# loicland/superpoint_graph

Hardware: NVIDIA H100
Metric: spg_train_step_edges_plus_points_per_sec (higher is better)
Workload: dtype f32

## Files before the change

### superpoint_graph_b200/csrc/tc_common.cuh

```cuda
#pragma once
#include <cuda_runtime.h>
#include <stdint.h>

namespace spg {

__device__ __forceinline__ uint32_t smem_u32(const void* p) {
    return (uint32_t)__cvta_generic_to_shared(p);
}

__device__ __forceinline__ uint32_t to_tf32(float v) {
    return (__float_as_uint(v) + 0x1000u) & 0xffffe000u;
}

__device__ __forceinline__ void mbar_init(uint32_t bar, uint32_t count) {
    asm volatile("mbarrier.init.shared::cta.b64 [%0], %1;" ::"r"(bar), "r"(count));
}

__device__ __forceinline__ void mbar_wait(uint32_t bar, uint32_t parity) {
    asm volatile(
        "{\n\t"
        ".reg .pred P1;\n\t"
        "WAIT_LOOP:\n\t"
        "mbarrier.try_wait.parity.shared::cta.b64 P1, [%0], %1;\n\t"
        "@P1 bra WAIT_DONE;\n\t"
        "bra WAIT_LOOP;\n\t"
        "WAIT_DONE:\n\t"
        "}" ::"r"(bar), "r"(parity)
        : "memory");
}

__device__ __forceinline__ void mbar_arrive(uint32_t bar) {
    asm volatile("mbarrier.arrive.shared::cta.b64 _, [%0];" ::"r"(bar) : "memory");
}

__device__ __forceinline__ void mbar_expect_tx(uint32_t bar, uint32_t bytes) {
    asm volatile("mbarrier.arrive.expect_tx.shared::cta.b64 _, [%0], %1;" ::"r"(bar), "r"(bytes) : "memory");
}

__device__ __forceinline__ uint64_t wg_desc_k_sw128(uint32_t saddr) {
    return (uint64_t)((saddr >> 4) & 0x3FFFu) | ((uint64_t)1 << 16) | ((uint64_t)64 << 32) | ((uint64_t)1 << 62);
}

__device__ __forceinline__ uint32_t sw128_off(int row, int c16) {
    return (uint32_t)((row >> 3) * 1024 + (row & 7) * 128 + ((c16 ^ (row & 7)) << 4));
}

__device__ __forceinline__ void wg_fence() { asm volatile("wgmma.fence.sync.aligned;" ::: "memory"); }
__device__ __forceinline__ void wg_commit() { asm volatile("wgmma.commit_group.sync.aligned;" ::: "memory"); }
template <int N>
__device__ __forceinline__ void wg_wait() {
    asm volatile("wgmma.wait_group.sync.aligned %0;" ::"n"(N) : "memory");
}

template <int R>
__device__ __forceinline__ void wg_reg_fence(float (&d)[R]) {
#pragma unroll
    for (int i = 0; i < R; ++i) asm volatile("" : "+f"(d[i])::"memory");
}

template <int N>
__device__ __forceinline__ void wgmma_tf32(float (&d)[N / 2], uint64_t da, uint64_t db, uint32_t acc);
template <int N>
__device__ __forceinline__ void wgmma_bf16(float (&d)[N / 2], uint64_t da, uint64_t db, uint32_t acc);

template <>
__device__ __forceinline__ void wgmma_tf32<16>(float (&d)[8], uint64_t da, uint64_t db, uint32_t acc) {
    asm volatile(
        "{\n\t.reg .pred p;\n\tsetp.ne.b32 p, %10, 0;\n\t"
        "wgmma.mma_async.sync.aligned.m64n16k8.f32.tf32.tf32 {%0, %1, %2, %3, %4, %5, %6, %7}, %8, %9, p, 1, 1;\n\t}"
        : "+f"(d[0]), "+f"(d[1]), "+f"(d[2]), "+f"(d[3]), "+f"(d[4]), "+f"(d[5]), "+f"(d[6]), "+f"(d[7])
        : "l"(da), "l"(db), "r"(acc));
}

template <>
__device__ __forceinline__ void wgmma_tf32<32>(float (&d)[16], uint64_t da, uint64_t db, uint32_t acc) {
    asm volatile(
        "{\n\t.reg .pred p;\n\tsetp.ne.b32 p, %18, 0;\n\t"
        "wgmma.mma_async.sync.aligned.m64n32k8.f32.tf32.tf32 {%0, %1, %2, %3, %4, %5, %6, %7, %8, %9, %10, %11, %12, %13, %14, %15}, %16, %17, p, 1, 1;\n\t}"
        : "+f"(d[0]), "+f"(d[1]), "+f"(d[2]), "+f"(d[3]), "+f"(d[4]), "+f"(d[5]), "+f"(d[6]), "+f"(d[7]), "+f"(d[8]), "+f"(d[9]), "+f"(d[10]), "+f"(d[11]), "+f"(d[12]), "+f"(d[13]), "+f"(d[14]), "+f"(d[15])
        : "l"(da), "l"(db), "r"(acc));
}

template <>
__device__ __forceinline__ void wgmma_tf32<64>(float (&d)[32], uint64_t da, uint64_t db, uint32_t acc) {
    asm volatile(
        "{\n\t.reg .pred p;\n\tsetp.ne.b32 p, %34, 0;\n\t"
        "wgmma.mma_async.sync.aligned.m64n64k8.f32.tf32.tf32 {%0, %1, %2, %3, %4, %5, %6, %7, %8, %9, %10, %11, %12, %13, %14, %15, %16, %17, %18, %19, %20, %21, %22, %23, %24, %25, %26, %27, %28, %29, %30, %31}, %32, %33, p, 1, 1;\n\t}"
        : "+f"(d[0]), "+f"(d[1]), "+f"(d[2]), "+f"(d[3]), "+f"(d[4]), "+f"(d[5]), "+f"(d[6]), "+f"(d[7]), "+f"(d[8]), "+f"(d[9]), "+f"(d[10]), "+f"(d[11]), "+f"(d[12]), "+f"(d[13]), "+f"(d[14]), "+f"(d[15]), "+f"(d[16]), "+f"(d[17]), "+f"(d[18]), "+f"(d[19]), "+f"(d[20]), "+f"(d[21]), "+f"(d[22]), "+f"(d[23]), "+f"(d[24]), "+f"(d[25]), "+f"(d[26]), "+f"(d[27]), "+f"(d[28]), "+f"(d[29]), "+f"(d[30]), "+f"(d[31])
        : "l"(da), "l"(db), "r"(acc));
}

template <>
__device__ __forceinline__ void wgmma_tf32<128>(float (&d)[64], uint64_t da, uint64_t db, uint32_t acc) {
    asm volatile(
        "{\n\t.reg .pred p;\n\tsetp.ne.b32 p, %66, 0;\n\t"
        "wgmma.mma_async.sync.aligned.m64n128k8.f32.tf32.tf32 {%0, %1, %2, %3, %4, %5, %6, %7, %8, %9, %10, %11, %12, %13, %14, %15, %16, %17, %18, %19, %20, %21, %22, %23, %24, %25, %26, %27, %28, %29, %30, %31, %32, %33, %34, %35, %36, %37, %38, %39, %40, %41, %42, %43, %44, %45, %46, %47, %48, %49, %50, %51, %52, %53, %54, %55, %56, %57, %58, %59, %60, %61, %62, %63}, %64, %65, p, 1, 1;\n\t}"
        : "+f"(d[0]), "+f"(d[1]), "+f"(d[2]), "+f"(d[3]), "+f"(d[4]), "+f"(d[5]), "+f"(d[6]), "+f"(d[7]), "+f"(d[8]), "+f"(d[9]), "+f"(d[10]), "+f"(d[11]), "+f"(d[12]), "+f"(d[13]), "+f"(d[14]), "+f"(d[15]), "+f"(d[16]), "+f"(d[17]), "+f"(d[18]), "+f"(d[19]), "+f"(d[20]), "+f"(d[21]), "+f"(d[22]), "+f"(d[23]), "+f"(d[24]), "+f"(d[25]), "+f"(d[26]), "+f"(d[27]), "+f"(d[28]), "+f"(d[29]), "+f"(d[30]), "+f"(d[31]), "+f"(d[32]), "+f"(d[33]), "+f"(d[34]), "+f"(d[35]), "+f"(d[36]), "+f"(d[37]), "+f"(d[38]), "+f"(d[39]), "+f"(d[40]), "+f"(d[41]), "+f"(d[42]), "+f"(d[43]), "+f"(d[44]), "+f"(d[45]), "+f"(d[46]), "+f"(d[47]), "+f"(d[48]), "+f"(d[49]), "+f"(d[50]), "+f"(d[51]), "+f"(d[52]), "+f"(d[53]), "+f"(d[54]), "+f"(d[55]), "+f"(d[56]), "+f"(d[57]), "+f"(d[58]), "+f"(d[59]), "+f"(d[60]), "+f"(d[61]), "+f"(d[62]), "+f"(d[63])
        : "l"(da), "l"(db), "r"(acc));
}

template <>
__device__ __forceinline__ void wgmma_bf16<32>(float (&d)[16], uint64_t da, uint64_t db, uint32_t acc) {
    asm volatile(
        "{\n\t.reg .pred p;\n\tsetp.ne.b32 p, %18, 0;\n\t"
        "wgmma.mma_async.sync.aligned.m64n32k16.f32.bf16.bf16 {%0, %1, %2, %3, %4, %5, %6, %7, %8, %9, %10, %11, %12, %13, %14, %15}, %16, %17, p, 1, 1, 0, 0;\n\t}"
        : "+f"(d[0]), "+f"(d[1]), "+f"(d[2]), "+f"(d[3]), "+f"(d[4]), "+f"(d[5]), "+f"(d[6]), "+f"(d[7]), "+f"(d[8]), "+f"(d[9]), "+f"(d[10]), "+f"(d[11]), "+f"(d[12]), "+f"(d[13]), "+f"(d[14]), "+f"(d[15])
        : "l"(da), "l"(db), "r"(acc));
}

template <>
__device__ __forceinline__ void wgmma_bf16<64>(float (&d)[32], uint64_t da, uint64_t db, uint32_t acc) {
    asm volatile(
        "{\n\t.reg .pred p;\n\tsetp.ne.b32 p, %34, 0;\n\t"
        "wgmma.mma_async.sync.aligned.m64n64k16.f32.bf16.bf16 {%0, %1, %2, %3, %4, %5, %6, %7, %8, %9, %10, %11, %12, %13, %14, %15, %16, %17, %18, %19, %20, %21, %22, %23, %24, %25, %26, %27, %28, %29, %30, %31}, %32, %33, p, 1, 1, 0, 0;\n\t}"
        : "+f"(d[0]), "+f"(d[1]), "+f"(d[2]), "+f"(d[3]), "+f"(d[4]), "+f"(d[5]), "+f"(d[6]), "+f"(d[7]), "+f"(d[8]), "+f"(d[9]), "+f"(d[10]), "+f"(d[11]), "+f"(d[12]), "+f"(d[13]), "+f"(d[14]), "+f"(d[15]), "+f"(d[16]), "+f"(d[17]), "+f"(d[18]), "+f"(d[19]), "+f"(d[20]), "+f"(d[21]), "+f"(d[22]), "+f"(d[23]), "+f"(d[24]), "+f"(d[25]), "+f"(d[26]), "+f"(d[27]), "+f"(d[28]), "+f"(d[29]), "+f"(d[30]), "+f"(d[31])
        : "l"(da), "l"(db), "r"(acc));
}

template <>
__device__ __forceinline__ void wgmma_bf16<128>(float (&d)[64], uint64_t da, uint64_t db, uint32_t acc) {
    asm volatile(
        "{\n\t.reg .pred p;\n\tsetp.ne.b32 p, %66, 0;\n\t"
        "wgmma.mma_async.sync.aligned.m64n128k16.f32.bf16.bf16 {%0, %1, %2, %3, %4, %5, %6, %7, %8, %9, %10, %11, %12, %13, %14, %15, %16, %17, %18, %19, %20, %21, %22, %23, %24, %25, %26, %27, %28, %29, %30, %31, %32, %33, %34, %35, %36, %37, %38, %39, %40, %41, %42, %43, %44, %45, %46, %47, %48, %49, %50, %51, %52, %53, %54, %55, %56, %57, %58, %59, %60, %61, %62, %63}, %64, %65, p, 1, 1, 0, 0;\n\t}"
        : "+f"(d[0]), "+f"(d[1]), "+f"(d[2]), "+f"(d[3]), "+f"(d[4]), "+f"(d[5]), "+f"(d[6]), "+f"(d[7]), "+f"(d[8]), "+f"(d[9]), "+f"(d[10]), "+f"(d[11]), "+f"(d[12]), "+f"(d[13]), "+f"(d[14]), "+f"(d[15]), "+f"(d[16]), "+f"(d[17]), "+f"(d[18]), "+f"(d[19]), "+f"(d[20]), "+f"(d[21]), "+f"(d[22]), "+f"(d[23]), "+f"(d[24]), "+f"(d[25]), "+f"(d[26]), "+f"(d[27]), "+f"(d[28]), "+f"(d[29]), "+f"(d[30]), "+f"(d[31]), "+f"(d[32]), "+f"(d[33]), "+f"(d[34]), "+f"(d[35]), "+f"(d[36]), "+f"(d[37]), "+f"(d[38]), "+f"(d[39]), "+f"(d[40]), "+f"(d[41]), "+f"(d[42]), "+f"(d[43]), "+f"(d[44]), "+f"(d[45]), "+f"(d[46]), "+f"(d[47]), "+f"(d[48]), "+f"(d[49]), "+f"(d[50]), "+f"(d[51]), "+f"(d[52]), "+f"(d[53]), "+f"(d[54]), "+f"(d[55]), "+f"(d[56]), "+f"(d[57]), "+f"(d[58]), "+f"(d[59]), "+f"(d[60]), "+f"(d[61]), "+f"(d[62]), "+f"(d[63])
        : "l"(da), "l"(db), "r"(acc));
}


}
```

### superpoint_graph_b200/csrc/tc_dw.cu

```cuda
#include "common.cuh"
#include "tc_common.cuh"

namespace spg {

constexpr int DW_THREADS = 256;
constexpr int DW_PTS = 32;

struct DwArgs {
    const float* dY;
    int64_t lddy;
    const float* P;
    int64_t ldp;
    const float *p_scale, *p_shift;
    int p_relu;
    float* partial;
    int64_t M;
    int64_t pts_per_cta;
};

template <int CO, int CI>
__global__ void __launch_bounds__(DW_THREADS, 1) tc_dw_kernel(const DwArgs p) {
    constexpr int WM = CO >= 128 ? CO / 2 : 64;
    constexpr int WN = CO >= 128 ? CI : CI / 2;
    constexpr int MSUB = WM / 64;
    constexpr int A_BYTES = CO * DW_PTS * 4;
    constexpr int B_BYTES = CI * DW_PTS * 4;
    constexpr int STAGE_BYTES = 2 * A_BYTES + 2 * B_BYTES;
    static_assert(CO % 64 == 0 && CI % 32 == 0 && CI <= 128 && CO <= 256, "shape");
    constexpr int A_F4 = CO * DW_PTS / 4 / DW_THREADS;
    constexpr int B_F4 = CI * DW_PTS / 4 / DW_THREADS;

    extern __shared__ __align__(1024) uint8_t smem_raw[];
    uint8_t* smem = reinterpret_cast<uint8_t*>((reinterpret_cast<uintptr_t>(smem_raw) + 1023) & ~(uintptr_t)1023);

    const int t = threadIdx.x;
    const int warp = t >> 5, lane = t & 31;
    const int g = warp >> 2, wl = warp & 3;
    SPG_PDL_ENTRY();

    const int64_t m_beg = (int64_t)blockIdx.x * p.pts_per_cta;
    const int64_t m_end = min(p.M, m_beg + p.pts_per_cta);
    const int nchunks = m_beg < m_end ? (int)((m_end - m_beg + DW_PTS - 1) / DW_PTS) : 0;
    const bool pro = p.p_scale || p.p_shift || p.p_relu;

    auto coord = [](int i, int c4s, int& pt, int& c4) {
        const int wi = i >> 5, l = i & 31;
        pt = (wi & 3) * 8 + (l & 7);
        c4 = (wi >> 2) * 4 + (l >> 3);
        (void)c4s;
    };
    float4 ra[A_F4], rb[B_F4];
    auto load_chunk = [&](int ch) {
        const int64_t mrow = m_beg + (int64_t)ch * DW_PTS;
#pragma unroll
        for (int j = 0; j < A_F4; ++j) {
            int pt, c4;
            coord(t + DW_THREADS * j, CO / 4, pt, c4);
            ra[j] = (mrow + pt < m_end)
                        ? __ldg(reinterpret_cast<const float4*>(p.dY + (mrow + pt) * p.lddy + c4 * 4))
                        : make_float4(0.f, 0.f, 0.f, 0.f);
        }
#pragma unroll
        for (int j = 0; j < B_F4; ++j) {
            int pt, c4;
            coord(t + DW_THREADS * j, CI / 4, pt, c4);
            rb[j] = (mrow + pt < m_end)
                        ? __ldg(reinterpret_cast<const float4*>(p.P + (mrow + pt) * p.ldp + c4 * 4))
                        : make_float4(0.f, 0.f, 0.f, 0.f);
        }
    };
    auto split_store = [&](uint8_t* hi_base, uint8_t* lo_base, int pt, int c4, float4 v) {
        const float vv[4] = {v.x, v.y, v.z, v.w};
#pragma unroll
        for (int e = 0; e < 4; ++e) {
            const uint32_t off = sw128_off(4 * c4 + e, pt >> 2) + (uint32_t)(pt & 3) * 4u;
            const uint32_t hi = to_tf32(vv[e]);
            *reinterpret_cast<uint32_t*>(hi_base + off) = hi;
            *reinterpret_cast<uint32_t*>(lo_base + off) = to_tf32(vv[e] - __uint_as_float(hi));
        }
    };

    float acc[MSUB][WN / 2];
#pragma unroll
    for (int m = 0; m < MSUB; ++m)
#pragma unroll
        for (int i = 0; i < WN / 2; ++i) acc[m][i] = 0.f;
    const int row_g = CO >= 128 ? g * WM : 0;
    const int col_g = CO >= 128 ? 0 : g * WN;

    if (nchunks > 0) load_chunk(0);
    for (int ch = 0; ch < nchunks; ++ch) {
        const int s = ch & 1;
        uint8_t* stage = smem + (size_t)s * STAGE_BYTES;
        uint8_t* a_hi = stage;
        uint8_t* a_lo = stage + A_BYTES;
        uint8_t* b_hi = stage + 2 * A_BYTES;
        uint8_t* b_lo = b_hi + B_BYTES;
        wg_wait<1>();
        wg_reg_fence(acc[0]);
        if (MSUB > 1) wg_reg_fence(acc[MSUB - 1]);
        __syncthreads();
        const int64_t mrow = m_beg + (int64_t)ch * DW_PTS;
#pragma unroll
        for (int j = 0; j < A_F4; ++j) {
            int pt, c4;
            coord(t + DW_THREADS * j, CO / 4, pt, c4);
            split_store(a_hi, a_lo, pt, c4, ra[j]);
        }
#pragma unroll
        for (int j = 0; j < B_F4; ++j) {
            int pt, c4;
            coord(t + DW_THREADS * j, CI / 4, pt, c4);
            float4 v = rb[j];
            if (pro && (mrow + pt < m_end)) {
                float4 sc = make_float4(1.f, 1.f, 1.f, 1.f), sh = make_float4(0.f, 0.f, 0.f, 0.f);
                if (p.p_scale) sc = __ldg(reinterpret_cast<const float4*>(p.p_scale + c4 * 4));
                if (p.p_shift) sh = __ldg(reinterpret_cast<const float4*>(p.p_shift + c4 * 4));
                v.x = fmaf(v.x, sc.x, sh.x);
                v.y = fmaf(v.y, sc.y, sh.y);
                v.z = fmaf(v.z, sc.z, sh.z);
                v.w = fmaf(v.w, sc.w, sh.w);
                if (p.p_relu) {
                    v.x = fmaxf(v.x, 0.f);
                    v.y = fmaxf(v.y, 0.f);
                    v.z = fmaxf(v.z, 0.f);
                    v.w = fmaxf(v.w, 0.f);
                }
            }
            split_store(b_hi, b_lo, pt, c4, v);
        }
        asm volatile("fence.proxy.async.shared::cta;" ::: "memory");
        __syncthreads();
        {
            const uint32_t ah = smem_u32(a_hi) + (uint32_t)row_g * 128u, al = smem_u32(a_lo) + (uint32_t)row_g * 128u;
            const uint32_t bh = smem_u32(b_hi) + (uint32_t)col_g * 128u, bl = smem_u32(b_lo) + (uint32_t)col_g * 128u;
#pragma unroll
            for (int m = 0; m < MSUB; ++m) wg_reg_fence(acc[m]);
            wg_fence();
#pragma unroll
            for (int kb = 0; kb < DW_PTS / 8; ++kb) {
                const uint64_t dbh = wg_desc_k_sw128(bh + kb * 32), dbl = wg_desc_k_sw128(bl + kb * 32);
#pragma unroll
                for (int m = 0; m < MSUB; ++m) {
                    const uint64_t dah = wg_desc_k_sw128(ah + m * 64 * 128 + kb * 32);
                    const uint64_t dal = wg_desc_k_sw128(al + m * 64 * 128 + kb * 32);
                    wgmma_tf32<WN>(acc[m], dah, dbh, 1u);
                    wgmma_tf32<WN>(acc[m], dal, dbh, 1u);
                    wgmma_tf32<WN>(acc[m], dah, dbl, 1u);
                }
            }
            wg_commit();
        }
        if (ch + 1 < nchunks) load_chunk(ch + 1);
    }
    wg_wait<0>();
#pragma unroll
    for (int m = 0; m < MSUB; ++m) wg_reg_fence(acc[m]);

    float* out = p.partial + (int64_t)blockIdx.x * CO * CI;
    const int r = lane >> 2, cq = 2 * (lane & 3);
#pragma unroll
    for (int m = 0; m < MSUB; ++m) {
        const int row = row_g + m * 64 + wl * 16 + r;
#pragma unroll
        for (int j = 0; j < WN / 8; ++j) {
            const int col = col_g + 8 * j + cq;
            *reinterpret_cast<float2*>(out + (int64_t)row * CI + col) = make_float2(acc[m][4 * j], acc[m][4 * j + 1]);
            *reinterpret_cast<float2*>(out + (int64_t)(row + 8) * CI + col) =
                make_float2(acc[m][4 * j + 2], acc[m][4 * j + 3]);
        }
    }
}

template <int CO, int CI>
static int launch_dw(const DwArgs& a, int ctas, cudaStream_t s) {
    constexpr int STAGE_BYTES = 2 * CO * DW_PTS * 4 + 2 * CI * DW_PTS * 4;
    const int smem = 2 * STAGE_BYTES + 1024;
    cudaError_t e = cudaFuncSetAttribute(tc_dw_kernel<CO, CI>, cudaFuncAttributeMaxDynamicSharedMemorySize, smem);
    if (e != cudaSuccess) return (int)e;
    SPG_LAUNCH(K_TC_DW, s, (tc_dw_kernel<CO, CI>), (unsigned)ctas, DW_THREADS, smem, a);
    return launch_status();
}

}

using namespace spg;

extern "C" {

int spg_tc_dw_supported(int64_t M, int co, int ci) {
    const bool co_ok = (co == 64 || co == 128 || co == 256);
    const bool ci_ok = (ci == 32 || ci == 64 || ci == 128);
    return (M >= DW_PTS && co_ok && ci_ok) ? 1 : 0;
}

int spg_tc_dw_ctas(int64_t M) {
    int64_t chunks = ceil_div64(M, DW_PTS);
    int64_t ctas = chunks < kNumSMs ? chunks : kNumSMs;
    return (int)(ctas < 1 ? 1 : ctas);
}

int spg_tc_dw(const float* dY, int64_t lddy, const float* P, int64_t ldp, const float* p_scale,
              const float* p_shift, int p_relu, float* dW, float* workspace, int64_t M, int co, int ci,
              spg_stream_t stream) {
    if (!dY || !P || !dW || !workspace || M <= 0) return SPG_E_BADARG;
    if (!spg_tc_dw_supported(M, co, ci)) return SPG_E_UNSUPPORTED;
    if ((lddy & 3) || (ldp & 3) || lddy < co || ldp < ci) return SPG_E_ALIGN;
    if (((uintptr_t)dY | (uintptr_t)P | (uintptr_t)workspace | (uintptr_t)p_scale | (uintptr_t)p_shift) & 15)
        return SPG_E_ALIGN;
    const int ctas = spg_tc_dw_ctas(M);
    DwArgs a;
    a.dY = dY; a.lddy = lddy; a.P = P; a.ldp = ldp; a.p_scale = p_scale; a.p_shift = p_shift;
    a.p_relu = p_relu; a.partial = workspace; a.M = M;
    cudaStream_t s = (cudaStream_t)stream;
    a.pts_per_cta = ceil_div64(ceil_div64(M, ctas), DW_PTS) * DW_PTS;
    int rc;
#define SPG_DW_CASE(CO_, CI_) \
    if (co == CO_ && ci == CI_) rc = launch_dw<CO_, CI_>(a, ctas, s); else
    SPG_DW_CASE(64, 32) SPG_DW_CASE(64, 64) SPG_DW_CASE(64, 128) SPG_DW_CASE(128, 32)
    SPG_DW_CASE(128, 64) SPG_DW_CASE(128, 128) SPG_DW_CASE(256, 32) SPG_DW_CASE(256, 64)
    SPG_DW_CASE(256, 128) rc = SPG_E_UNSUPPORTED;
#undef SPG_DW_CASE
    if (rc) return rc;
    return spg_splitk_reduce(workspace, ctas, co, ci, nullptr, dW, ci, stream);
}

}
```

Measured before the change: 42.61 million.

## Warp-specialize weight-gradient kernel with producer warps and mbarrier multi-stage ring

Splits the dW GEMM kernel into 256 producer threads that load, apply the scale/shift/ReLU prologue and write hi/lo TF32 splits into a multi-stage shared-memory ring, and 256 consumer threads that issue wgmma. Full/empty mbarriers replace the block-wide __syncthreads, and setmaxnreg moves registers from producers to consumers. The intent is to overlap global loads and conversion with tensor-core work instead of serialising them per chunk. In exchange it doubles the thread count, uses much more shared memory, and adds barrier protocol complexity.

```diff
diff --git a/superpoint_graph_b200/csrc/tc_common.cuh b/superpoint_graph_b200/csrc/tc_common.cuh
--- a/superpoint_graph_b200/csrc/tc_common.cuh
+++ b/superpoint_graph_b200/csrc/tc_common.cuh
@@ -43,6 +43,15 @@
 
 __device__ __forceinline__ uint32_t sw128_off(int row, int c16) {
     return (uint32_t)((row >> 3) * 1024 + (row & 7) * 128 + ((c16 ^ (row & 7)) << 4));
+}
+
+template <int R>
+__device__ __forceinline__ void reg_budget_inc() {
+    asm volatile("setmaxnreg.inc.sync.aligned.u32 %0;" ::"n"(R));
+}
+template <int R>
+__device__ __forceinline__ void reg_budget_dec() {
+    asm volatile("setmaxnreg.dec.sync.aligned.u32 %0;" ::"n"(R));
 }
 
 __device__ __forceinline__ void wg_fence() { asm volatile("wgmma.fence.sync.aligned;" ::: "memory"); }
diff --git a/superpoint_graph_b200/csrc/tc_dw.cu b/superpoint_graph_b200/csrc/tc_dw.cu
--- a/superpoint_graph_b200/csrc/tc_dw.cu
+++ b/superpoint_graph_b200/csrc/tc_dw.cu
@@ -3,8 +3,27 @@
 
 namespace spg {
 
-constexpr int DW_THREADS = 256;
 constexpr int DW_PTS = 32;
+constexpr int DW_CONS_THREADS = 256, DW_PROD_THREADS = 256;
+constexpr int DW_THREADS = DW_CONS_THREADS + DW_PROD_THREADS;
+constexpr int DW_MAX_STAGES = 4;
+constexpr int DW_RING_BYTES = 232448 - 2048;
+
+template <int CO, int CI>
+struct DwShape {
+    static constexpr int A_BYTES = CO * DW_PTS * 4;
+    static constexpr int B_BYTES = CI * DW_PTS * 4;
+    static constexpr int STAGE_BYTES = 2 * A_BYTES + 2 * B_BYTES;
+    static constexpr int STAGES = DW_RING_BYTES / STAGE_BYTES < DW_MAX_STAGES ? DW_RING_BYTES / STAGE_BYTES
+                                                                            : DW_MAX_STAGES;
+    static constexpr int SMEM = STAGES * STAGE_BYTES + 2 * CI * 4 + 1024;
+    static_assert(STAGES >= 2, "ring");
+    static constexpr int ACC_REGS = CO >= 128 ? CO * CI / 256 : CI / 4;
+    static constexpr bool WIDE_ACC = ACC_REGS > 64;
+    static constexpr int PF = WIDE_ACC ? 3 : 4;
+    static constexpr int CONS_REGS = WIDE_ACC ? 160 : 144;
+    static constexpr int PROD_REGS = WIDE_ACC ? 96 : 112;
+};
 
 struct DwArgs {
     const float* dY;
@@ -18,68 +37,164 @@
     int64_t pts_per_cta;
 };
 
+__device__ __forceinline__ void st_shared4(uint32_t addr, uint4 v) {
+    asm volatile("st.shared.v4.b32 [%0], {%1, %2, %3, %4};" ::"r"(addr), "r"(v.x), "r"(v.y), "r"(v.z), "r"(v.w)
+                 : "memory");
+}
+
+__device__ __forceinline__ float f4_at(const float4& v, int e) { return e == 0 ? v.x : e == 1 ? v.y : e == 2 ? v.z : v.w; }
+
 template <int CO, int CI>
 __global__ void __launch_bounds__(DW_THREADS, 1) tc_dw_kernel(const DwArgs p) {
+    using S = DwShape<CO, CI>;
+    constexpr int STAGES = S::STAGES, PF = S::PF;
     constexpr int WM = CO >= 128 ? CO / 2 : 64;
     constexpr int WN = CO >= 128 ? CI : CI / 2;
     constexpr int MSUB = WM / 64;
-    constexpr int A_BYTES = CO * DW_PTS * 4;
-    constexpr int B_BYTES = CI * DW_PTS * 4;
-    constexpr int STAGE_BYTES = 2 * A_BYTES + 2 * B_BYTES;
+    constexpr int NB = 2 * (CO + CI);
+    constexpr int PROD_WARPS = NB / 32 < 8 ? NB / 32 : 8;
     static_assert(CO % 64 == 0 && CI % 32 == 0 && CI <= 128 && CO <= 256, "shape");
-    constexpr int A_F4 = CO * DW_PTS / 4 / DW_THREADS;
-    constexpr int B_F4 = CI * DW_PTS / 4 / DW_THREADS;
 
     extern __shared__ __align__(1024) uint8_t smem_raw[];
     uint8_t* smem = reinterpret_cast<uint8_t*>((reinterpret_cast<uintptr_t>(smem_raw) + 1023) & ~(uintptr_t)1023);
+    float* sc_s = reinterpret_cast<float*>(smem + (size_t)STAGES * S::STAGE_BYTES);
+    float* sh_s = sc_s + CI;
+    __shared__ __align__(8) uint64_t bars[2 * STAGES];
 
     const int t = threadIdx.x;
     const int warp = t >> 5, lane = t & 31;
-    const int g = warp >> 2, wl = warp & 3;
+    const uint32_t smem_u = smem_u32(smem);
+    const uint32_t bars_u32 = smem_u32(&bars[0]);
+    auto bar_full = [&](int s) { return bars_u32 + 8u * (uint32_t)s; };
+    auto bar_empty = [&](int s) { return bars_u32 + 8u * (uint32_t)(STAGES + s); };
+    if (t == 0) {
+#pragma unroll
+        for (int s = 0; s < STAGES; ++s) {
+            mbar_init(bar_full(s), PROD_WARPS);
+            mbar_init(bar_empty(s), DW_CONS_THREADS / 32);
+        }
+        asm volatile("fence.mbarrier_init.release.cluster;" ::: "memory");
+    }
     SPG_PDL_ENTRY();
 
     const int64_t m_beg = (int64_t)blockIdx.x * p.pts_per_cta;
     const int64_t m_end = min(p.M, m_beg + p.pts_per_cta);
     const int nchunks = m_beg < m_end ? (int)((m_end - m_beg + DW_PTS - 1) / DW_PTS) : 0;
+
+    const int pt = t - DW_CONS_THREADS;
+    const int nbt = pt >= 0 && pt < NB ? (NB - pt + DW_PROD_THREADS - 1) / DW_PROD_THREADS : 0;
+    float4 q[PF][4];
+    auto load = [&](int ch, int j, float4 (&dst)[4]) {
+        if (ch >= nchunks) return;
+        const int b = pt + DW_PROD_THREADS * j;
+        const bool is_a = b < 2 * CO;
+        const int bl = is_a ? b : b - 2 * CO;
+        const int64_t ld = is_a ? p.lddy : p.ldp;
+        const int64_t row0 = m_beg + (int64_t)ch * DW_PTS + 4 * (bl & 7);
+        const float* src = (is_a ? p.dY : p.P) + row0 * ld + 4 * (bl >> 3);
+#pragma unroll
+        for (int r = 0; r < 4; ++r) {
+            float4 v = make_float4(0.f, 0.f, 0.f, 0.f);
+            if (row0 + r < m_end)
+                asm volatile("ld.global.nc.L1::no_allocate.L2::256B.v4.f32 {%0, %1, %2, %3}, [%4];"
+                             : "=f"(v.x), "=f"(v.y), "=f"(v.z), "=f"(v.w)
+                             : "l"(src + r * ld));
+            dst[r] = v;
+        }
+    };
+    auto advance = [&](int& ch, int& j) {
+        if (++j == nbt) {
+            j = 0;
+            ++ch;
+        }
+    };
+    int lch = 0, lj = 0;
+    if (nbt > 0) {
+#pragma unroll
+        for (int d = 0; d < PF - 1; ++d) {
+            load(lch, lj, q[d]);
+            advance(lch, lj);
+        }
+    }
     const bool pro = p.p_scale || p.p_shift || p.p_relu;
-
-    auto coord = [](int i, int c4s, int& pt, int& c4) {
-        const int wi = i >> 5, l = i & 31;
-        pt = (wi & 3) * 8 + (l & 7);
-        c4 = (wi >> 2) * 4 + (l >> 3);
-        (void)c4s;
-    };
-    float4 ra[A_F4], rb[B_F4];
-    auto load_chunk = [&](int ch) {
-        const int64_t mrow = m_beg + (int64_t)ch * DW_PTS;
-#pragma unroll
-        for (int j = 0; j < A_F4; ++j) {
-            int pt, c4;
-            coord(t + DW_THREADS * j, CO / 4, pt, c4);
-            ra[j] = (mrow + pt < m_end)
-                        ? __ldg(reinterpret_cast<const float4*>(p.dY + (mrow + pt) * p.lddy + c4 * 4))
-                        : make_float4(0.f, 0.f, 0.f, 0.f);
-        }
-#pragma unroll
-        for (int j = 0; j < B_F4; ++j) {
-            int pt, c4;
-            coord(t + DW_THREADS * j, CI / 4, pt, c4);
-            rb[j] = (mrow + pt < m_end)
-                        ? __ldg(reinterpret_cast<const float4*>(p.P + (mrow + pt) * p.ldp + c4 * 4))
-                        : make_float4(0.f, 0.f, 0.f, 0.f);
-        }
-    };
-    auto split_store = [&](uint8_t* hi_base, uint8_t* lo_base, int pt, int c4, float4 v) {
-        const float vv[4] = {v.x, v.y, v.z, v.w};
-#pragma unroll
-        for (int e = 0; e < 4; ++e) {
-            const uint32_t off = sw128_off(4 * c4 + e, pt >> 2) + (uint32_t)(pt & 3) * 4u;
-            const uint32_t hi = to_tf32(vv[e]);
-            *reinterpret_cast<uint32_t*>(hi_base + off) = hi;
-            *reinterpret_cast<uint32_t*>(lo_base + off) = to_tf32(vv[e] - __uint_as_float(hi));
-        }
-    };
-
+    for (int i = t; i < CI; i += DW_THREADS) {
+        sc_s[i] = p.p_scale ? p.p_scale[i] : 1.f;
+        sh_s[i] = p.p_shift ? p.p_shift[i] : 0.f;
+    }
+    __syncthreads();
+
+    if (warp >= DW_CONS_THREADS / 32) {
+        reg_budget_dec<S::PROD_REGS>();
+        if (nbt == 0) return;
+        int ch = 0, j = 0;
+        auto store = [&](const float4 (&v0)[4]) {
+            const int s = ch % STAGES;
+            if (j == 0 && ch >= STAGES) mbar_wait(bar_empty(s), (uint32_t)((ch / STAGES - 1) & 1));
+            const int b = pt + DW_PROD_THREADS * j;
+            const bool is_a = b < 2 * CO;
+            const int bl = is_a ? b : b - 2 * CO;
+            const int c16 = bl & 7, c4 = bl >> 3;
+            float4 v[4] = {v0[0], v0[1], v0[2], v0[3]};
+            if (!is_a && pro) {
+                const float4 sc = *reinterpret_cast<const float4*>(sc_s + 4 * c4);
+                const float4 sh = *reinterpret_cast<const float4*>(sh_s + 4 * c4);
+                const int64_t row0 = m_beg + (int64_t)ch * DW_PTS + 4 * c16;
+#pragma unroll
+                for (int r = 0; r < 4; ++r) {
+                    if (row0 + r < m_end) {
+                        v[r].x = fmaf(v[r].x, sc.x, sh.x);
+                        v[r].y = fmaf(v[r].y, sc.y, sh.y);
+                        v[r].z = fmaf(v[r].z, sc.z, sh.z);
+                        v[r].w = fmaf(v[r].w, sc.w, sh.w);
+                        if (p.p_relu) {
+                            v[r].x = fmaxf(v[r].x, 0.f);
+                            v[r].y = fmaxf(v[r].y, 0.f);
+                            v[r].z = fmaxf(v[r].z, 0.f);
+                            v[r].w = fmaxf(v[r].w, 0.f);
+                        }
+                    }
+                }
+            }
+            const uint32_t hi_base = smem_u + (uint32_t)(s * S::STAGE_BYTES + (is_a ? 0 : 2 * S::A_BYTES));
+            const uint32_t lo_base = hi_base + (uint32_t)(is_a ? S::A_BYTES : S::B_BYTES);
+#pragma unroll
+            for (int e = 0; e < 4; ++e) {
+                uint4 hi, lo;
+                hi.x = to_tf32(f4_at(v[0], e));
+                hi.y = to_tf32(f4_at(v[1], e));
+                hi.z = to_tf32(f4_at(v[2], e));
+                hi.w = to_tf32(f4_at(v[3], e));
+                lo.x = to_tf32(f4_at(v[0], e) - __uint_as_float(hi.x));
+                lo.y = to_tf32(f4_at(v[1], e) - __uint_as_float(hi.y));
+                lo.z = to_tf32(f4_at(v[2], e) - __uint_as_float(hi.z));
+                lo.w = to_tf32(f4_at(v[3], e) - __uint_as_float(hi.w));
+                const uint32_t off = sw128_off(4 * c4 + e, c16);
+                st_shared4(hi_base + off, hi);
+                st_shared4(lo_base + off, lo);
+            }
+            if (j == nbt - 1) {
+                asm volatile("fence.proxy.async.shared::cta;" ::: "memory");
+                __syncwarp();
+                if (lane == 0) mbar_arrive(bar_full(s));
+            }
+            advance(ch, j);
+        };
+        const int total = nchunks * nbt;
+        int item = 0;
+        while (item < total) {
+#pragma unroll
+            for (int u = 0; u < PF; ++u) {
+                load(lch, lj, q[(u + PF - 1) % PF]);
+                advance(lch, lj);
+                store(q[u]);
+                if (++item >= total) break;
+            }
+        }
+        return;
+    }
+
+    reg_budget_inc<S::CONS_REGS>();
+    const int g = warp >> 2, wl = warp & 3;
     float acc[MSUB][WN / 2];
 #pragma unroll
     for (int m = 0; m < MSUB; ++m)
@@ -87,71 +202,38 @@
         for (int i = 0; i < WN / 2; ++i) acc[m][i] = 0.f;
     const int row_g = CO >= 128 ? g * WM : 0;
     const int col_g = CO >= 128 ? 0 : g * WN;
-
-    if (nchunks > 0) load_chunk(0);
+    int prev = -1;
     for (int ch = 0; ch < nchunks; ++ch) {
-        const int s = ch & 1;
-        uint8_t* stage = smem + (size_t)s * STAGE_BYTES;
-        uint8_t* a_hi = stage;
-        uint8_t* a_lo = stage + A_BYTES;
-        uint8_t* b_hi = stage + 2 * A_BYTES;
-        uint8_t* b_lo = b_hi + B_BYTES;
+        const int s = ch % STAGES;
+        mbar_wait(bar_full(s), (uint32_t)((ch / STAGES) & 1));
+        const uint32_t ah = smem_u + (uint32_t)(s * S::STAGE_BYTES + row_g * 128);
+        const uint32_t al = ah + S::A_BYTES;
+        const uint32_t bh = smem_u + (uint32_t)(s * S::STAGE_BYTES + 2 * S::A_BYTES + col_g * 128);
+        const uint32_t bl = bh + S::B_BYTES;
+#pragma unroll
+        for (int m = 0; m < MSUB; ++m) wg_reg_fence(acc[m]);
+        wg_fence();
+#pragma unroll
+        for (int kb = 0; kb < DW_PTS / 8; ++kb) {
+            const uint64_t dbh = wg_desc_k_sw128(bh + kb * 32), dbl = wg_desc_k_sw128(bl + kb * 32);
+#pragma unroll
+            for (int m = 0; m < MSUB; ++m) {
+                const uint64_t dah = wg_desc_k_sw128(ah + m * 64 * 128 + kb * 32);
+                const uint64_t dal = wg_desc_k_sw128(al + m * 64 * 128 + kb * 32);
+                wgmma_tf32<WN>(acc[m], dah, dbh, 1u);
+                wgmma_tf32<WN>(acc[m], dal, dbh, 1u);
+                wgmma_tf32<WN>(acc[m], dah, dbl, 1u);
+            }
+        }
+        wg_commit();
         wg_wait<1>();
-        wg_reg_fence(acc[0]);
-        if (MSUB > 1) wg_reg_fence(acc[MSUB - 1]);
-        __syncthreads();
-        const int64_t mrow = m_beg + (int64_t)ch * DW_PTS;
-#pragma unroll
-        for (int j = 0; j < A_F4; ++j) {
-            int pt, c4;
-            coord(t + DW_THREADS * j, CO / 4, pt, c4);
-            split_store(a_hi, a_lo, pt, c4, ra[j]);
-        }
-#pragma unroll
-        for (int j = 0; j < B_F4; ++j) {
-            int pt, c4;
-            coord(t + DW_THREADS * j, CI / 4, pt, c4);
-            float4 v = rb[j];
-            if (pro && (mrow + pt < m_end)) {
-                float4 sc = make_float4(1.f, 1.f, 1.f, 1.f), sh = make_float4(0.f, 0.f, 0.f, 0.f);
-                if (p.p_scale) sc = __ldg(reinterpret_cast<const float4*>(p.p_scale + c4 * 4));
-                if (p.p_shift) sh = __ldg(reinterpret_cast<const float4*>(p.p_shift + c4 * 4));
-                v.x = fmaf(v.x, sc.x, sh.x);
-                v.y = fmaf(v.y, sc.y, sh.y);
-                v.z = fmaf(v.z, sc.z, sh.z);
-                v.w = fmaf(v.w, sc.w, sh.w);
-                if (p.p_relu) {
-                    v.x = fmaxf(v.x, 0.f);
-                    v.y = fmaxf(v.y, 0.f);
-                    v.z = fmaxf(v.z, 0.f);
-                    v.w = fmaxf(v.w, 0.f);
-                }
-            }
-            split_store(b_hi, b_lo, pt, c4, v);
-        }
-        asm volatile("fence.proxy.async.shared::cta;" ::: "memory");
-        __syncthreads();
-        {
-            const uint32_t ah = smem_u32(a_hi) + (uint32_t)row_g * 128u, al = smem_u32(a_lo) + (uint32_t)row_g * 128u;
-            const uint32_t bh = smem_u32(b_hi) + (uint32_t)col_g * 128u, bl = smem_u32(b_lo) + (uint32_t)col_g * 128u;
-#pragma unroll
-            for (int m = 0; m < MSUB; ++m) wg_reg_fence(acc[m]);
-            wg_fence();
-#pragma unroll
-            for (int kb = 0; kb < DW_PTS / 8; ++kb) {
-                const uint64_t dbh = wg_desc_k_sw128(bh + kb * 32), dbl = wg_desc_k_sw128(bl + kb * 32);
-#pragma unroll
-                for (int m = 0; m < MSUB; ++m) {
-                    const uint64_t dah = wg_desc_k_sw128(ah + m * 64 * 128 + kb * 32);
-                    const uint64_t dal = wg_desc_k_sw128(al + m * 64 * 128 + kb * 32);
-                    wgmma_tf32<WN>(acc[m], dah, dbh, 1u);
-                    wgmma_tf32<WN>(acc[m], dal, dbh, 1u);
-                    wgmma_tf32<WN>(acc[m], dah, dbl, 1u);
-                }
-            }
-            wg_commit();
-        }
-        if (ch + 1 < nchunks) load_chunk(ch + 1);
+#pragma unroll
+        for (int m = 0; m < MSUB; ++m) wg_reg_fence(acc[m]);
+        if (prev >= 0) {
+            __syncwarp();
+            if (lane == 0) mbar_arrive(bar_empty(prev));
+        }
+        prev = s;
     }
     wg_wait<0>();
 #pragma unroll
@@ -174,8 +256,7 @@
 
 template <int CO, int CI>
 static int launch_dw(const DwArgs& a, int ctas, cudaStream_t s) {
-    constexpr int STAGE_BYTES = 2 * CO * DW_PTS * 4 + 2 * CI * DW_PTS * 4;
-    const int smem = 2 * STAGE_BYTES + 1024;
+    const int smem = DwShape<CO, CI>::SMEM;
     cudaError_t e = cudaFuncSetAttribute(tc_dw_kernel<CO, CI>, cudaFuncAttributeMaxDynamicSharedMemorySize, smem);
     if (e != cudaSuccess) return (int)e;
     SPG_LAUNCH(K_TC_DW, s, (tc_dw_kernel<CO, CI>), (unsigned)ctas, DW_THREADS, smem, a);
```

After: 44.42 million (median of 6 runs). +4.2%, better.
